# pangenome/impg

Hardware: AMD Instinct MI355X
Metric: projected ranges/sec, 1M-PAF 100k-BED -x depth 3; CPU coitrees baseline (higher is better)
Workload: dtype int32

## Files before the change

impg_amd/csrc/kernels.hip:

```cpp
#include <hip/hip_runtime.h>

#include <cstring>

#include "device_prims.hpp"
#include "impg_internal.hpp"
#include "kernels.hpp"

namespace impg {

__device__ __forceinline__ unsigned lane_id() { return threadIdx.x & 63u; }
__device__ __forceinline__ unsigned long long lanemask_lt() { return (1ull << lane_id()) - 1ull; }

template <int CTRL, int ROW_MASK>
__device__ __forceinline__ uint32_t dpp_or0(uint32_t x) {
  return (uint32_t)__builtin_amdgcn_update_dpp(0, (int)x, CTRL, ROW_MASK, 0xF, false);
}
__device__ __forceinline__ uint32_t wave_incl_scan(uint32_t x) {
  x += dpp_or0<0x111, 0xF>(x);
  x += dpp_or0<0x112, 0xF>(x);
  x += dpp_or0<0x114, 0xF>(x);
  x += dpp_or0<0x118, 0xF>(x);
  x += dpp_or0<0x142, 0xA>(x);
  x += dpp_or0<0x143, 0xC>(x);
  return x;
// ... 1462 lines not shown
};
constexpr uint32_t PROJ_WL_WORDS = 65u + 3u;
constexpr uint32_t PROJ_RG_WORDS = PROJ_BLOCK + 4u * PROJ_BLOCK + PROJ_WAVES + (4u - PROJ_WAVES % 4u) % 4u;
__device__ __forceinline__ PairIn pair_of_place(uint32_t pp, uint32_t lblock, uint32_t n_pairs, const FrontierRec *__restrict__ fr,
                                                const uint32_t *__restrict__ pair_range, const uint32_t *__restrict__ pair_entry,
                                                const ProjList &pl, const WindowLists &wl, uint32_t *wl_off ) {
  PairIn x;
  x.live = pp < n_pairs;
  x.p = pp; x.eidx = 0xFFFFFFFFu; x.f_start = 0; x.f_end = 0;
  uint32_t r = 0;
  if (wl.tile_first && lblock * PROJ_BLOCK >= n_pairs) {
  } else if (wl.tile_first) {
    const uint32_t pp_last = min(lblock * PROJ_BLOCK + PROJ_BLOCK, n_pairs) - 1u;
    uint32_t base_i = wl.tile_first[lblock], ri = 0, k = 0;
    bool found = !x.live;
    for (;;) {
      if (threadIdx.x < 65u) wl_off[threadIdx.x] = base_i + threadIdx.x < wl.n_fr ? wl.pair_off[base_i + threadIdx.x] : 0xFFFFFFFFu;
      __syncthreads();
      const uint32_t lim = wl_off[64];
      if (!found && pp < lim) {
        uint32_t j = 0;
#pragma unroll
        for (uint32_t st = 32u; st > 0u; st >>= 1) j += wl_off[j + st] <= pp ? st : 0u;
        ri = base_i + j;
        k = pp - wl_off[j];
        found = true;
      }
      __syncthreads();
      if (lim > pp_last) break;
      base_i += 64u;
    }
    if (x.live) {
      const uint4 w = wl.win[ri];
      const FrontierRec sf = wl.se[ri];
      const int2 se = make_int2(sf.start, sf.end);
      x.f_start = se.x; x.f_end = se.y;
      if (w.y - (w.x & ~3u) > 64u) x.eidx = pair_entry[pp];
      else x.eidx = w.x + select_bit64(w.z, w.w, k);
      if (wl.range_out) wl.range_out[pp] = wl.range_places ? ri : wl.perm[ri];
    }
  } else if (x.live) {
    if (pl.slot) { x.p = pl.slot[pp]; r = pl.range[pp]; x.eidx = pl.entry[pp]; }
    else { r = pair_range[pp]; x.eidx = pair_entry[pp]; }
    asm volatile("" : "+v"(r), "+v"(x.eidx));
    const FrontierRec f = fr[r];
    x.f_start = f.start; x.f_end = f.end;
  }
  return x;
}
template <uint32_t NB>
__device__ __forceinline__ void regroup_by_entry(PairIn &x, uint32_t *scratch ) {
  uint4 *rg_pay = reinterpret_cast<uint4 *>(scratch);
  uint32_t *rg_hist = scratch + 4u * NB, *rg_ws = rg_hist + NB;
  rg_hist[threadIdx.x] = 0u;
  __syncthreads();
  const uint32_t bin = x.eidx & (NB - 1u);
  const uint32_t pos = atomicAdd(&rg_hist[bin], 1u);
  __syncthreads();
  {
    const uint32_t cnt = rg_hist[threadIdx.x], inc = wave_incl_scan(cnt);
    if (lane_id() == 63u) rg_ws[threadIdx.x >> 6] = inc;
    __syncthreads();
    uint32_t base = 0;
#pragma unroll
    for (uint32_t k = 0; k + 1u < NB / 64u; k++) base += k < (threadIdx.x >> 6) ? rg_ws[k] : 0u;
    rg_hist[threadIdx.x] = base + inc - cnt;
  }
  __syncthreads();
  rg_pay[rg_hist[bin] + pos] = make_uint4(x.eidx, x.p, (uint32_t)x.f_start, (uint32_t)x.f_end);
  __syncthreads();
  const uint4 mine = rg_pay[threadIdx.x];
  x.eidx = mine.x; x.p = mine.y; x.f_start = (int32_t)mine.z; x.f_end = (int32_t)mine.w;
  x.live = x.eidx != 0xFFFFFFFFu;
}
template <uint32_t NW>
__device__ __forceinline__ void count_accepted(uint32_t mine, unsigned long long *__restrict__ accepted, uint32_t *wcnt ) {
  uint32_t w = mine;
#pragma unroll
  for (int o = 32; o > 0; o >>= 1) w += __shfl_xor(w, o);
  if (lane_id() == 0) wcnt[threadIdx.x >> 6] = w;
  __syncthreads();
  if (threadIdx.x == 0) {
    uint32_t tot = 0;
#pragma unroll
    for (uint32_t k = 0; k < NW; k++) tot += wcnt[k];
    if (tot) atomicAdd(&accepted[(blockIdx.x % COUNT_SLOTS) * COUNT_STRIDE], (unsigned long long)tot);
  }
}
template <bool TRANSITIVE, int MODE>
__global__ __launch_bounds__(PROJ_BLOCK) void project_kernel(DeviceIndexView v, const FrontierRec *__restrict__ fr,
                                                      const uint32_t *__restrict__ pair_range,
                                                      const uint32_t *__restrict__ pair_entry, uint32_t n_pairs,
                                                      HitArrays h, unsigned long long *__restrict__ accepted,
                                                      uint32_t *__restrict__ err_flag, double min_identity,
                                                      SliceArrays sl, ProjList pl, int xcd_map,
                                                      const uint32_t *__restrict__ n_pairs_dev, int regroup, WindowLists wl) {
  if (n_pairs_dev) n_pairs = *n_pairs_dev;
  const uint32_t per_xcd = gridDim.x >> 3;
  const uint32_t lblock = xcd_map ? (blockIdx.x & 7u) * per_xcd + (blockIdx.x >> 3) : blockIdx.x;
  const uint32_t pp = lblock * PROJ_BLOCK + threadIdx.x;
#ifdef IMPG_PHASE_CLOCKS
  unsigned long long phase_t[10];
  for (int i = 0; i < 10; i++) phase_t[i] = 0;
  PHASE_MARK(0);
#endif
  bool ok = false;
  TileScan res;
  res.found = res.any = false;
  res.pqs = res.pts = res.pqe = res.pte = -1;
  uint32_t qid = HIT_NONE;
  __shared__ uint32_t wl_off[PROJ_WL_WORDS];
  __shared__ uint4 rg_scratch[PROJ_RG_WORDS / 4u];
  __shared__ uint32_t wcnt[PROJ_WAVES];
  PairIn x = pair_of_place(pp, lblock, n_pairs, fr, pair_range, pair_entry, pl, wl, wl_off);
  PHASE_MARK(1);
  if (regroup) regroup_by_entry<PROJ_BLOCK>(x, reinterpret_cast<uint32_t *>(rg_scratch));
  PHASE_MARK(2);
  if (x.live) {
    project_pair<TRANSITIVE, MODE>(v, x.eidx, x.f_start, x.f_end, x.p, min_identity, err_flag, sl, accepted, ok, qid, res PHASE_PASS);
    h.qid[x.p] = qid;
    if (ok) {
      h.c[x.p] = make_int4(res.pqs, res.pqe, res.pts, res.pte);
    }
  }
  PHASE_MARK(7);
  count_accepted<PROJ_WAVES>(ok ? 1u : 0u, accepted, wcnt);
#ifdef IMPG_PHASE_CLOCKS
  PHASE_MARK(8);
  if ((blockIdx.x & 63u) == 0u && lane_id() == 0u && phase_t[3] && phase_t[4] && phase_t[5] && phase_t[6]) {
    for (int i = 0; i < 8; i++) atomicAdd(&g_phase_clk[i], phase_t[i + 1] - phase_t[i]);
    atomicAdd(&g_phase_clk[15], 1ull);
  }
#endif
}

#ifndef IMPG_STG_THREADS
#define IMPG_STG_THREADS 512
#endif
#ifndef IMPG_STG_RANGES
#define IMPG_STG_RANGES 256
#endif
#ifndef IMPG_STG_ECAP
#define IMPG_STG_ECAP 56
#endif
constexpr uint32_t STG_THREADS = IMPG_STG_THREADS, STG_WAVES = STG_THREADS / 64u;
constexpr uint32_t STG_RANGES = IMPG_STG_RANGES;
constexpr uint32_t STG_ECAP = IMPG_STG_ECAP;
constexpr uint32_t STG_ENT_V4 = STG_ECAP * STG_ENT_STRIDE / 4u;
constexpr uint32_t STG_LINE_V4 = STG_ECAP * STG_REC_STRIDE / 4u;
static_assert((STG_RANGES & (STG_RANGES - 1u)) == 0u && STG_RANGES < STG_THREADS && STG_THREADS % 64u == 0, "a thread per range, whole waves");
static_assert(STG_LINE_V4 * 4u >= 5u * STG_THREADS + STG_WAVES, "the unstaged path's scratch overlays the line buffer");
static_assert(STG_ECAP * 4u <= STG_THREADS, "one pass copies the entries");
constexpr int OUT_SLOTS = 0, OUT_QS = 1, OUT_ROWS = 2;
template <bool TRANSITIVE, bool MASKS, bool CAN_STAGE = true, uint32_t NR = STG_RANGES, uint32_t NT = STG_THREADS, int MODE = 0, int OUT = OUT_SLOTS>
__device__ __forceinline__ uint32_t project_places(const DeviceIndexView &v, const uint32_t *__restrict__ pair_entry, const HitArrays &h,
                                                   unsigned long long *__restrict__ accepted, uint32_t *__restrict__ err_flag,
                                                   const WindowLists &wl, uint32_t r0, uint32_t P0, uint32_t P1, uint32_t emin, uint32_t n_e,
                                                   bool regroup_all, const uint32_t *st_off, const uint4 *st_win, const int2 *st_se,
                                                   const uint4 *st_ent, uint4 *st_line PHASE_ARG, double min_identity = 0.0,
                                                   const uint32_t *st_dest = nullptr, const uint32_t *st_tid = nullptr) {
  const SliceArrays no_sl{nullptr, nullptr, nullptr, nullptr};
  uint32_t n_ok = 0;
  constexpr bool ordered = OUT == OUT_ROWS;
  constexpr bool qs = OUT == OUT_QS;
  if (ordered || qs) regroup_all = false;
  uint32_t e_next = 0xFFFFFFFFu;
  if (!MASKS && (unsigned long long)P0 + threadIdx.x < P1) e_next = pair_entry[P0 + threadIdx.x];
  const bool by_visit = ordered && MASKS && wl.ord.by_visit != 0u;
  uint32_t v_next = 0u;
  if (by_visit && (unsigned long long)P0 + threadIdx.x < P1) v_next = wl.ord.vpos[P0 + threadIdx.x];
#pragma unroll 1
  for (uint32_t base = P0; base < P1; base += NT) {
    if (base + NT < base) break;
    const uint32_t pp = base + threadIdx.x;
    PairIn y;
    y.live = pp < P1 ? 1u : 0u;
    y.p = pp; y.eidx = 0xFFFFFFFFu; y.f_start = 0; y.f_end = 0;
    uint32_t j = 0;
#pragma unroll
    for (uint32_t st = NR / 2u; st > 0u; st >>= 1) j += st_off[j + st] <= pp ? st : 0u;
    uint32_t o_dest = 0, o_tid = 0;
    if (y.live) {
      const int2 se = st_se[j];
      y.f_start = se.x; y.f_end = se.y;
      if (MASKS) {
        const uint4 w = st_win[j];
        const bool listed = w.y - (w.x & ~3u) > 64u;
        if (listed) y.eidx = pair_entry[pp];
        else if (by_visit) y.eidx = w.x + v_next;
        else y.eidx = w.x + select_bit64(w.z, w.w, pp - st_off[j]);
        if (ordered) {
          o_dest = st_dest[j] + (listed || by_visit ? pp - st_off[j] : (uint32_t)wl.ord.vpos[pp]);
          o_tid = st_tid ? st_tid[j] : wl.se[r0 + j].target_id;
        } else if (qs) o_tid = r0 + j;
        else if (wl.range_out) wl.range_out[pp] = wl.range_places ? r0 + j : wl.perm[r0 + j];
      } else {
        y.eidx = e_next;
      }
    }
    if (!MASKS) {
      e_next = 0xFFFFFFFFu;
      if ((unsigned long long)pp + NT < P1) e_next = pair_entry[pp + NT];
    }
    if (by_visit) {
      v_next = 0u;
      if ((unsigned long long)pp + NT < P1) v_next = wl.ord.vpos[pp + NT];
    }
    if (regroup_all) regroup_by_entry<NT>(y, reinterpret_cast<uint32_t *>(st_line));
    if (y.live) {
      bool ok = false;
      TileScan res;
      res.found = res.any = false;
      res.pqs = res.pts = res.pqe = res.pte = -1;
      uint32_t qid = HIT_NONE;
      const uint32_t slot = y.eidx - emin;
      const uint4 *se = st_ent + min(slot, STG_ECAP - 1u) * (STG_ENT_STRIDE / 4u);
      if (CAN_STAGE && slot < n_e && (se[1].z & OP_LEN_MASK) <= INLINE_TILES * TILE_OPS)
        project_pair<TRANSITIVE, MODE, true>(v, y.eidx, y.f_start, y.f_end, y.p, min_identity, err_flag, no_sl, accepted, ok, qid, res PHASE_PASS, se,
                                             reinterpret_cast<const uint32_t *>(st_line + slot * (STG_REC_STRIDE / 4u)));
      else
        project_pair<TRANSITIVE, MODE>(v, y.eidx, y.f_start, y.f_end, y.p, min_identity, err_flag, no_sl, accepted, ok, qid, res PHASE_PASS);
      if (ordered) put_ordered_row(wl.ord, o_dest, qid, o_tid, ok, res.pqs, res.pqe, res.pts, res.pte);
      else {
        if (qs) reinterpret_cast<uint2 *>(h.qid)[y.p] = make_uint2(qid, o_tid);
        else h.qid[y.p] = qid;
        if (ok) h.c[y.p] = make_int4(res.pqs, res.pqe, res.pts, res.pte);
      }
      n_ok += ok ? 1u : 0u;
    }
    if (regroup_all) __syncthreads();
  }
  return n_ok;
}
template <bool TRANSITIVE, bool MASKS, int OUT = OUT_SLOTS>
__global__ __launch_bounds__(STG_THREADS) void project_staged_kernel(DeviceIndexView v, const uint32_t *__restrict__ pair_entry,
                                                      uint32_t n_pairs, HitArrays h, unsigned long long *__restrict__ accepted,
                                                      uint32_t *__restrict__ err_flag, int regroup, WindowLists wl) {
  const uint32_t per_xcd = gridDim.x >> 3;
  const uint32_t sblock = (blockIdx.x & 7u) * per_xcd + (blockIdx.x >> 3);
  __shared__ uint4 st_ent[STG_ENT_V4];
  __shared__ uint4 st_line[STG_LINE_V4];
  __shared__ uint4 st_win[STG_RANGES];
  __shared__ int2 st_se[STG_RANGES];
  __shared__ uint32_t st_off[STG_RANGES + 4u];
  __shared__ uint32_t st_dest[OUT == OUT_ROWS ? STG_RANGES : 1u], st_tid[OUT == OUT_ROWS ? STG_RANGES : 1u];
  __shared__ uint32_t wred[2u * STG_WAVES];
  __shared__ uint32_t wcnt[STG_WAVES];
  const uint32_t r0 = sblock * STG_RANGES;
  if (r0 >= wl.n_fr) return;
  const uint32_t nr = min(STG_RANGES, wl.n_fr - r0);
  if (OUT == OUT_ROWS && threadIdx.x < nr) st_dest[threadIdx.x] = wl.ord.dest[r0 + threadIdx.x];
#ifdef IMPG_PHASE_CLOCKS
  unsigned long long stg_t[8], phase_t[10];
#define STG_MARK(i) do { asm volatile("s_waitcnt vmcnt(0) lgkmcnt(0)" ::: "memory"); stg_t[i] = __builtin_readcyclecounter(); } while (0)
#else
#define STG_MARK(i) do { } while (0)
#endif
  STG_MARK(0);
  uint32_t emin = 0xFFFFFFFFu, emax = 0u;
  if (threadIdx.x <= STG_RANGES) {
    uint32_t o = 0xFFFFFFFFu;
    if (threadIdx.x < nr) o = wl.pair_off[r0 + threadIdx.x];
    else if (threadIdx.x == nr) o = r0 + nr < wl.n_fr ? wl.pair_off[r0 + nr] : n_pairs;
    st_off[threadIdx.x] = o;
    if (threadIdx.x < nr) {
      const uint4 w = wl.win[r0 + threadIdx.x];
      st_win[threadIdx.x] = w;
      { const FrontierRec sf = wl.se[r0 + threadIdx.x]; st_se[threadIdx.x] = make_int2(sf.start, sf.end); if (OUT == OUT_ROWS) st_tid[threadIdx.x] = sf.target_id; }
      if (w.y - (w.x & ~3u) > 64u) { emin = w.x; emax = w.y - 1u; }
      else if (w.z | w.w) {
        emin = w.x + (w.z ? (uint32_t)__builtin_ctz(w.z) : 32u + (uint32_t)__builtin_ctz(w.w));
        emax = w.x + (w.w ? 63u - (uint32_t)__builtin_clz(w.w) : 31u - (uint32_t)__builtin_clz(w.z));
      }
    }
  }
  {
#pragma unroll
    for (int o = 32; o > 0; o >>= 1) {
      emin = min(emin, (uint32_t)__shfl_xor((int)emin, o));
      emax = max(emax, (uint32_t)__shfl_xor((int)emax, o));
    }
    if (lane_id() == 0) { wred[threadIdx.x >> 6] = emin; wred[STG_WAVES + (threadIdx.x >> 6)] = emax; }
    __syncthreads();
#pragma unroll
    for (uint32_t k = 0; k < STG_WAVES; k++) { emin = min(emin, wred[k]); emax = max(emax, wred[STG_WAVES + k]); }
  }
  const uint32_t P0 = st_off[0], P1 = st_off[nr];
  uint32_t n_ok = 0;
  STG_MARK(1);
  const bool sparse = emin <= emax && emax - emin >= 4u * STG_ECAP;
  uint32_t n_e = 0;
  if (emin <= emax && !sparse) {
    n_e = min(STG_ECAP, emax - emin + 1u);
    if (threadIdx.x < n_e * 4u) st_ent[(threadIdx.x >> 2) * (STG_ENT_STRIDE / 4u) + (threadIdx.x & 3u)] = reinterpret_cast<const uint4 *>(v.entries + emin)[threadIdx.x];
    __syncthreads();
    const uint32_t w = threadIdx.x >> 6, l = lane_id();
    constexpr uint32_t TURNS = (STG_ECAP + STG_WAVES - 1u) / STG_WAVES;
    uint4 buf[TURNS];
#pragma unroll
    for (uint32_t k = 0; k < TURNS; k++) {
      const uint32_t i = w + k * STG_WAVES;
      buf[k] = make_uint4(0u, 0u, 0u, 0u);
      if (i < n_e) {
        const uint4 e1 = st_ent[i * (STG_ENT_STRIDE / 4u) + 1u];
        const uint32_t n = e1.z & OP_LEN_MASK, m = (n + TILE_OPS - 1u) / TILE_OPS;
        if (m <= INLINE_TILES && (l >> 3) < m) buf[k] = reinterpret_cast<const uint4 *>(v.pfx + (size_t)e1.y * TILE_WORDS)[l];
      }
    }
#pragma unroll
    for (uint32_t k = 0; k < TURNS; k++) {
      const uint32_t i = w + k * STG_WAVES;
      if (i < n_e) st_line[i * (STG_REC_STRIDE / 4u) + (l >> 3) * (STG_LINE_STRIDE / 4u) + (l & 7u)] = buf[k];
    }
    __syncthreads();
  }
  STG_MARK(2);
  n_ok = project_places<TRANSITIVE, MASKS, true, STG_RANGES, STG_THREADS, 0, OUT>(v, pair_entry, h, accepted, err_flag, wl, r0, P0, P1, emin, n_e,
                                                                                  sparse && regroup != 0, st_off, st_win, st_se, st_ent, st_line PHASE_PASS,
                                                                                  0.0, st_dest, OUT == OUT_ROWS ? st_tid : nullptr);
#ifdef IMPG_PHASE_CLOCKS
  STG_MARK(3);
  if ((blockIdx.x & 15u) == 0u && threadIdx.x == 0u) {
    if (sparse) {
      atomicAdd(&g_phase_clk[13], stg_t[3] - stg_t[0]);
      atomicAdd(&g_phase_clk[14], 1ull);
      atomicAdd(&g_phase_clk[12], (unsigned long long)(emax - emin));
    } else {
      for (int i = 0; i < 3; i++) atomicAdd(&g_phase_clk[i], stg_t[i + 1] - stg_t[i]);
      atomicAdd(&g_phase_clk[9], (unsigned long long)(P1 - P0));
      atomicAdd(&g_phase_clk[10], emin <= emax && emax - emin >= STG_ECAP ? 1ull : 0ull);
      atomicAdd(&g_phase_clk[15], 1ull);
      atomicAdd(&g_phase_clk[11], emin <= emax ? (unsigned long long)(emax - emin + 1u) : 0ull);
    }
  }
#endif
  count_accepted<STG_WAVES>(n_ok, accepted, wcnt);
}
#undef STG_MARK

#ifndef IMPG_ENT_RANGES
#define IMPG_ENT_RANGES 512
#endif
#ifndef IMPG_ENT_THREADS
#define IMPG_ENT_THREADS 256
#endif
constexpr uint32_t ENT_RANGES = IMPG_ENT_RANGES;
constexpr uint32_t ENT_THREADS = IMPG_ENT_THREADS, ENT_WAVES = ENT_THREADS / 64u;
constexpr uint32_t ENT_REC_STRIDE = ENT_CP_OFF + 16u;
static_assert((ENT_RANGES & (ENT_RANGES - 1u)) == 0u && ENT_RANGES % ENT_THREADS == 0 && ENT_THREADS % 64u == 0, "whole turns of the block over its ranges");
constexpr uint32_t ENT_REC_V4 = ENT_WAVES * ENT_REC_STRIDE / 4u, ENT_LIST_V4 = ENT_WAVES * ENT_RANGES * 2u / 16u;
static_assert((ENT_REC_V4 + ENT_LIST_V4) * 4u >= 5u * ENT_THREADS + ENT_WAVES, "the unstaged path's scratch overlays the waves' records and lists");
#ifndef IMPG_ENT_WAVES
#define IMPG_ENT_WAVES 6
#endif
template <bool TRANSITIVE, int ORIENT, int MODE, int OUT>
__device__ __forceinline__ void project_entry_chunk(const DeviceIndexView &v, uint4 e0, uint4 e1, uint4 e2, uint4 e3, uint32_t eidx, bool live,
                                                    int32_t f_start, int32_t f_end, uint32_t p, const uint32_t *rec, const HitArrays &h,
                                                    unsigned long long *__restrict__ accepted, uint32_t *__restrict__ err_flag,
                                                    uint32_t &n_ok PHASE_ARG, double min_identity, const OrderedOut &ord, uint32_t tid) {
  const SliceArrays no_sl{nullptr, nullptr, nullptr, nullptr};
  if (live) {
    bool ok = false;
    TileScan res;
    res.found = res.any = false;
    res.pqs = res.pts = res.pqe = res.pte = -1;
    uint32_t qid = HIT_NONE;
    if (ORIENT >= 0) {
      e0 = reinterpret_cast<const uint4 *>(__builtin_assume_aligned(rec, 16))[ENT_CP_OFF / 4u + 3u];
      asm volatile("" : "+v"(e0.x), "+v"(e0.y), "+v"(e0.z), "+v"(e0.w));
    }
    if (ORIENT >= 0)
      project_core<TRANSITIVE, MODE, true, ORIENT>(v, e0, e1, e2, e3, f_start, f_end, p, min_identity, err_flag, no_sl, accepted, ok, qid, res PHASE_PASS, rec);
    else
      project_pair<TRANSITIVE, MODE>(v, eidx, f_start, f_end, p, min_identity, err_flag, no_sl, accepted, ok, qid, res PHASE_PASS);
    if (OUT == OUT_ROWS) put_ordered_row(ord, p, qid, tid, ok, res.pqs, res.pqe, res.pts, res.pte);
    else {
      if (OUT == OUT_QS) reinterpret_cast<uint2 *>(h.qid)[p] = make_uint2(qid, tid);
      else h.qid[p] = qid;
      if (ok) h.c[p] = make_int4(res.pqs, res.pqe, res.pts, res.pte);
    }
    n_ok += ok ? 1u : 0u;
  }
}
#ifndef IMPG_ENT_SLICE_PAIRS
#define IMPG_ENT_SLICE_PAIRS 32768
#endif
constexpr uint32_t ENT_SLICE_PAIRS = IMPG_ENT_SLICE_PAIRS, ENT_MAX_SLICES = 64u;
#ifndef IMPG_ENT_SPARSE
#define IMPG_ENT_SPARSE 4
#endif
constexpr uint32_t ENT_SPARSE = IMPG_ENT_SPARSE;
struct EntSlices {
  uint32_t *work;
  uint32_t *alloc;
  uint32_t cap;
  int phase;
};
template <bool TRANSITIVE, int MODE, int OUT>
__global__ __launch_bounds__(ENT_THREADS) __attribute__((amdgpu_waves_per_eu(IMPG_ENT_WAVES, IMPG_ENT_WAVES)))
void project_entries_kernel(DeviceIndexView v, const uint32_t *__restrict__ pair_entry, uint32_t n_pairs,
                                                      HitArrays h, unsigned long long *__restrict__ accepted,
                                                      uint32_t *__restrict__ err_flag, int regroup, WindowLists wl, double min_identity, EntSlices sl) {
  const uint32_t per_xcd = gridDim.x >> 3;
  uint32_t sblock = (blockIdx.x & 7u) * per_xcd + (blockIdx.x >> 3);
  uint32_t slice = 0u, n_slices = 1u;
  if (sl.phase) {
    if (blockIdx.x >= min(sl.work[0], sl.cap)) return;
    const uint32_t item = sl.work[1u + blockIdx.x];
    sblock = item >> 12; slice = (item >> 6) & 63u; n_slices = (item & 63u) + 1u;
  }
  __shared__ uint4 st_work[ENT_REC_V4 + ENT_LIST_V4];
  uint4 (*st_rec)[ENT_REC_STRIDE / 4u] = reinterpret_cast<uint4 (*)[ENT_REC_STRIDE / 4u]>(st_work);
  uint16_t (*st_list)[ENT_RANGES] = reinterpret_cast<uint16_t (*)[ENT_RANGES]>(st_work + ENT_REC_V4);
  __shared__ uint4 st_win[ENT_RANGES];
  __shared__ int2 st_se[ENT_RANGES];
  __shared__ uint32_t st_off[ENT_RANGES + 4u];
  __shared__ uint16_t st_wide[ENT_RANGES];
  __shared__ uint32_t st_dest[OUT == OUT_ROWS ? ENT_RANGES : 1u];
  constexpr bool ordered = OUT == OUT_ROWS;
  constexpr bool qs = OUT == OUT_QS;
  constexpr bool WIDE_LISTED = ordered;
  __shared__ uint32_t st_nwide, st_alloc, st_next;
  __shared__ uint32_t wred[2u * ENT_WAVES];
  __shared__ uint32_t wcnt[ENT_WAVES];
  const uint32_t r0 = sblock * ENT_RANGES;
  if (r0 >= wl.n_fr) return;
  const uint32_t nr = min(ENT_RANGES, wl.n_fr - r0);
  const uint32_t wv = (uint32_t)__builtin_amdgcn_readfirstlane((int)(threadIdx.x >> 6)), l = lane_id();
#ifdef IMPG_PHASE_CLOCKS
  unsigned long long stg_t[8], phase_t[10];
#define STG_MARK(i) do { asm volatile("s_waitcnt vmcnt(0) lgkmcnt(0)" ::: "memory"); stg_t[i] = __builtin_readcyclecounter(); } while (0)
#else
#define STG_MARK(i) do { } while (0)
#endif
  STG_MARK(0);
  if (threadIdx.x == 0) { st_nwide = 0u; st_alloc = 0u; st_next = 0u; }
  __syncthreads();
  uint32_t emin = 0xFFFFFFFFu, emax = 0u;
#pragma unroll
  for (uint32_t t = threadIdx.x; t < ENT_RANGES; t += ENT_THREADS) {
    if (t < nr) st_off[t] = wl.pair_off[r0 + t];
    else st_off[t + 1u] = 0xFFFFFFFFu;
    if (t == 0) st_off[nr] = r0 + nr < wl.n_fr ? wl.pair_off[r0 + nr] : n_pairs;
    uint32_t glo = 0xFFFFFFFFu, ghi = 0u;
    if (t < nr) {
      const uint4 w = wl.win[r0 + t];
      st_win[t] = w;
      { const FrontierRec sf = wl.se[r0 + t]; st_se[t] = make_int2(sf.start, sf.end); }
      if (ordered) st_dest[t] = wl.ord.dest[r0 + t];
      if (w.y - (w.x & ~3u) > 64u) {
        if (WIDE_LISTED) st_wide[atomicAdd(&st_nwide, 1u)] = (uint16_t)t;
        else if (w.x < w.y) { glo = w.x; ghi = w.y - 1u; emin = min(emin, glo); emax = max(emax, ghi); }
      } else if (w.z | w.w) {
        glo = w.x + (w.z ? (uint32_t)__builtin_ctz(w.z) : 32u + (uint32_t)__builtin_ctz(w.w));
        ghi = w.x + (w.w ? 63u - (uint32_t)__builtin_clz(w.w) : 31u - (uint32_t)__builtin_clz(w.z));
        emin = min(emin, glo);
        emax = max(emax, ghi);
      }
    }
  }
  {
#pragma unroll
    for (int o = 32; o > 0; o >>= 1) {
      emin = min(emin, (uint32_t)__shfl_xor((int)emin, o));
      emax = max(emax, (uint32_t)__shfl_xor((int)emax, o));
    }
    if (l == 0) { wred[wv] = emin; wred[ENT_WAVES + wv] = emax; }
    __syncthreads();
#pragma unroll
    for (uint32_t k = 0; k < ENT_WAVES; k++) { emin = min(emin, wred[k]); emax = max(emax, wred[ENT_WAVES + k]); }
    emin = (uint32_t)__builtin_amdgcn_readfirstlane((int)emin);
    emax = (uint32_t)__builtin_amdgcn_readfirstlane((int)emax);
  }
  const uint32_t P0 = st_off[0], P1 = st_off[nr];
  const bool compact = !ordered;
  uint32_t n_ok = 0;
  STG_MARK(1);
  const bool sparse = emin <= emax && (unsigned long long)(P1 - P0) < (unsigned long long)ENT_SPARSE * (emax - emin + 1u);
  if (!sl.phase && sl.work && !sparse && emin <= emax && P1 - P0 > ENT_SLICE_PAIRS && (uint32_t)__builtin_amdgcn_readfirstlane((int)st_nwide) == 0u) {
    n_slices = min(ENT_MAX_SLICES, (P1 - P0 + ENT_SLICE_PAIRS - 1u) / ENT_SLICE_PAIRS);
    if (threadIdx.x == 0) {
      const uint32_t at = atomicAdd(&sl.work[0], n_slices - 1u);
      for (uint32_t k = 1; k < n_slices; k++)
        if (at + k - 1u < sl.cap) sl.work[1u + at + k - 1u] = sblock << 12 | k << 6 | (n_slices - 1u);
    }
  }
  if (sparse) {
    n_ok = project_places<TRANSITIVE, true, false, ENT_RANGES, ENT_THREADS, MODE, OUT>(v, pair_entry, h, accepted, err_flag, wl, r0, P0, P1, emin, 0u, regroup != 0, st_off, st_win,
                                                               st_se, nullptr, st_work PHASE_PASS, min_identity, st_dest);
  } else if (emin <= emax) {
    const uint4 *ents = reinterpret_cast<const uint4 *>(v.entries);
    const uint4 zero4 = make_uint4(0u, 0u, 0u, 0u);
    const uint32_t n_span = emax - emin + 1u;
    auto take = [&]() -> uint32_t {
      uint32_t i = 0;
      if (l == 0) i = atomicAdd(&st_next, 1u);
      i = (uint32_t)__builtin_amdgcn_readfirstlane((int)i);
      return n_slices > 1u ? min(n_span, slice + i * n_slices) : i;
    };
    uint32_t ic = take(), in = take();
    uint4 cq = zero4, nq = zero4, lc = zero4;
    auto fetch_entry = [&](uint32_t i) -> uint4 {
      uint4 q = zero4;
      if (i < n_span && l < 4u) q = ents[(size_t)(emin + i) * 4u + l];
      return q;
    };
#define IMPG_RDL(x, j) (uint32_t)__builtin_amdgcn_readlane((int)(x), j)
    auto fetch_record = [&](const uint4 &q) -> uint4 {
      uint4 r = zero4;
      const uint32_t nz = IMPG_RDL(q.z, 1), ny = IMPG_RDL(q.y, 1);
      const uint32_t m = ((nz & OP_LEN_MASK) + TILE_OPS - 1u) / TILE_OPS;
      if (m <= INLINE_TILES && (l >> 3) < m) r = reinterpret_cast<const uint4 *>(v.pfx + (size_t)ny * TILE_WORDS)[l];
      return r;
    };
    cq = fetch_entry(ic);
    nq = fetch_entry(in);
    if (ic < n_span) lc = fetch_record(cq);
#pragma unroll 1
    while (ic < n_span) {
      const uint32_t eidx = emin + ic;
      __builtin_amdgcn_wave_barrier();
      st_rec[wv][(l >> 3) * (STG_LINE_STRIDE / 4u) + (l & 7u)] = lc;
      if (l < 4u) st_rec[wv][ENT_CP_OFF / 4u + ((l + 3u) & 3u)] = cq;
      uint4 e0, e1, e2, e3;
      e0.x = IMPG_RDL(cq.x, 0); e0.y = IMPG_RDL(cq.y, 0); e0.z = IMPG_RDL(cq.z, 0); e0.w = IMPG_RDL(cq.w, 0);
      e1.x = IMPG_RDL(cq.x, 1); e1.y = IMPG_RDL(cq.y, 1); e1.z = IMPG_RDL(cq.z, 1); e1.w = IMPG_RDL(cq.w, 1);
      e2.x = IMPG_RDL(cq.x, 2); e2.y = IMPG_RDL(cq.y, 2); e2.z = IMPG_RDL(cq.z, 2); e2.w = IMPG_RDL(cq.w, 2);
      e3.x = IMPG_RDL(cq.x, 3); e3.y = IMPG_RDL(cq.y, 3); e3.z = IMPG_RDL(cq.z, 3); e3.w = IMPG_RDL(cq.w, 3);
      ic = in;
      cq = nq;
      lc = zero4;
      if (ic < n_span) {
        lc = fetch_record(cq);
        in = take();
        nq = fetch_entry(in);
      }
      uint32_t cnt = 0;
      const int32_t e_end = TRANSITIVE ? ((int32_t)e0.x < (int32_t)e0.y ? (int32_t)e0.y : (-2147483647 - 1)) : (int32_t)e0.y;
#pragma unroll
      for (uint32_t q = 0; q < ENT_RANGES / 64u; q++) {
        const uint32_t r = q * 64u + l;
        bool hit = false;
        if (r < nr) {
          const uint4 w = st_win[r];
          const uint32_t d = eidx - w.x;
          if (w.y - (w.x & ~3u) <= 64u) hit = d < 64u && (((d < 32u ? w.z >> d : w.w >> (d - 32u)) & 1u) != 0u);
          else if (!WIDE_LISTED) hit = eidx >= w.x && eidx < w.y && window_hit<TRANSITIVE>(e_end, st_se[r].x);
        }
        const unsigned long long b = __ballot(hit);
        if (hit) st_list[wv][cnt + (uint32_t)__popcll(b & lanemask_lt())] = (uint16_t)r;
        cnt += (uint32_t)__popcll(b);
      }
      uint32_t run = 0;
      if (compact) {
        if (l == 0) run = n_slices > 1u ? atomicAdd(&sl.alloc[sblock], cnt) : atomicAdd(&st_alloc, cnt);
        run = P0 + (uint32_t)__builtin_amdgcn_readfirstlane((int)run);
      }
      asm volatile("s_waitcnt lgkmcnt(0)" ::: "memory");
      __builtin_amdgcn_wave_barrier();
      const uint32_t *rec = reinterpret_cast<const uint32_t *>(&st_rec[wv][0]);
      const int orient = (e1.z & OP_LEN_MASK) > INLINE_TILES * TILE_OPS ? -1 : !(e1.z & EF_REVERSED) ? 0 : (e1.z & EF_STRAND) ? 2 : 1;
      uint32_t tid = 0;
      if (ordered && cnt) tid = wl.se[r0 + (uint32_t)__builtin_amdgcn_readfirstlane((int)st_list[wv][0])].target_id;
#pragma unroll 1
      for (uint32_t k0 = 0; k0 < cnt; k0 += 64u) {
        const bool live = k0 + l < cnt;
        const uint32_t r = live ? (uint32_t)st_list[wv][k0 + l] : 0u;
        const int2 se = st_se[r];
        uint32_t p = run + k0 + l;
        if (!compact) {
          const uint4 w = st_win[r];
          const uint32_t d = eidx - w.x;
          const uint32_t below = d < 32u ? (uint32_t)__popc(w.z & ((1u << d) - 1u))
                                         : (uint32_t)__popc(w.z) + (uint32_t)__popc(w.w & ((1u << (d - 32u)) - 1u));
          p = st_off[r] + below;
        }
        if (ordered) {
          if (live) p = st_dest[r] + (uint32_t)wl.ord.vpos[p];
        } else if (qs) tid = r0 + r;
        else if (live && wl.range_out) wl.range_out[p] = wl.range_places ? r0 + r : wl.perm[r0 + r];
        if (orient == 0) project_entry_chunk<TRANSITIVE, 0, MODE, OUT>(v, e0, e1, e2, e3, eidx, live, se.x, se.y, p, rec, h, accepted, err_flag, n_ok PHASE_PASS, min_identity, wl.ord, tid);
        else if (orient == 1) project_entry_chunk<TRANSITIVE, 1, MODE, OUT>(v, e0, e1, e2, e3, eidx, live, se.x, se.y, p, rec, h, accepted, err_flag, n_ok PHASE_PASS, min_identity, wl.ord, tid);
        else if (orient == 2) project_entry_chunk<TRANSITIVE, 2, MODE, OUT>(v, e0, e1, e2, e3, eidx, live, se.x, se.y, p, rec, h, accepted, err_flag, n_ok PHASE_PASS, min_identity, wl.ord, tid);
        else project_entry_chunk<TRANSITIVE, -1, MODE, OUT>(v, e0, e1, e2, e3, eidx, live, se.x, se.y, p, rec, h, accepted, err_flag, n_ok PHASE_PASS, min_identity, wl.ord, tid);
      }
    }
#undef IMPG_RDL
#ifdef IMPG_PHASE_CLOCKS
    STG_MARK(2);
    if ((blockIdx.x & 15u) == 0u && threadIdx.x == 0u) {
      atomicAdd(&g_phase_clk[0], stg_t[1] - stg_t[0]);
      atomicAdd(&g_phase_clk[2], stg_t[2] - stg_t[1]);
      atomicAdd(&g_phase_clk[9], (unsigned long long)(P1 - P0));
      atomicAdd(&g_phase_clk[15], 1ull);
      atomicAdd(&g_phase_clk[11], (unsigned long long)(emax - emin + 1u));
    }
#endif
  }
  if (!sparse) {
    const SliceArrays no_sl{nullptr, nullptr, nullptr, nullptr};
    const uint32_t nw = st_nwide;
#pragma unroll 1
    for (uint32_t k = 0; k < nw; k++) {
      const uint32_t r = st_wide[k];
      const uint32_t a = st_off[r], b = st_off[r + 1u];
      const int2 se = st_se[r];
#pragma unroll 1
      for (uint32_t pp = a + threadIdx.x; pp < b; pp += ENT_THREADS) {
        bool ok = false;
        TileScan res;
        res.found = res.any = false;
        res.pqs = res.pts = res.pqe = res.pte = -1;
        uint32_t qid = HIT_NONE;
        project_pair<TRANSITIVE, MODE>(v, pair_entry[pp], se.x, se.y, pp, min_identity, err_flag, no_sl, accepted, ok, qid, res PHASE_PASS);
        if (ordered)
          put_ordered_row(wl.ord, st_dest[r] + (pp - a), qid, wl.se[r0 + r].target_id, ok, res.pqs, res.pqe, res.pts, res.pte);
        else {
          if (qs) reinterpret_cast<uint2 *>(h.qid)[pp] = make_uint2(qid, r0 + r);
          else h.qid[pp] = qid;
          if (ok) h.c[pp] = make_int4(res.pqs, res.pqe, res.pts, res.pte);
        }
        n_ok += ok ? 1u : 0u;
        if (wl.range_out && !ordered && !qs) wl.range_out[pp] = wl.range_places ? r0 + r : wl.perm[r0 + r];
      }
    }
  }
#ifdef IMPG_PHASE_CLOCKS
  if (sparse && (blockIdx.x & 15u) == 0u && threadIdx.x == 0u) {
    STG_MARK(3);
    atomicAdd(&g_phase_clk[13], stg_t[3] - stg_t[0]);
    atomicAdd(&g_phase_clk[14], 1ull);
    atomicAdd(&g_phase_clk[12], (unsigned long long)(emax - emin));
  }
#endif
  count_accepted<ENT_WAVES>(n_ok, accepted, wcnt);
}
#undef STG_MARK
#ifdef IMPG_PHASE_CLOCKS
extern "C" void impg_gpu_debug_phase_clocks(unsigned long long *out) {
  unsigned long long z[16] = {};
  (void)hipDeviceSynchronize();
  (void)hipMemcpyFromSymbol(out, HIP_SYMBOL(g_phase_clk), sizeof(z));
  (void)hipMemcpyToSymbol(HIP_SYMBOL(g_phase_clk), z, sizeof(z));
}
#endif

__device__ __forceinline__ int32_t tp_refine(int32_t query_pos, int32_t query_delta, int32_t seg_start, int32_t overlap_pos,
                                             int32_t abs_target_delta, bool first, int32_t lo, int32_t hi) {
  int32_t refined;
  if (abs_target_delta == 0) {
    refined = first ? query_pos : query_pos + query_delta;
  } else {
    const double target_fraction = (double)(overlap_pos - seg_start) / (double)abs_target_delta;
    const double indel_ratio = (double)query_delta / (double)abs_target_delta;
    const double query_advance = target_fraction * (double)abs_target_delta * indel_ratio;
    const double r = round(query_advance);
    const int32_t adv = r >= 2147483647.0 ? 2147483647 : r <= -2147483648.0 ? (-2147483647 - 1) : (int32_t)r;
    refined = (int32_t)((uint32_t)query_pos + (uint32_t)adv);
  }
  return min(max(refined, lo), hi);
}
template <bool TRANSITIVE>
__global__ __launch_bounds__(256) void project_tp_kernel(DeviceIndexView v, const FrontierRec *__restrict__ fr,
                                                         const uint32_t *__restrict__ pair_range,
                                                         const uint32_t *__restrict__ pair_entry, uint32_t n_pairs,
                                                         HitArrays h, unsigned long long *__restrict__ accepted,
                                                         uint32_t *__restrict__ err_flag, double min_identity, int use_ident,
                                                         ProjList pl, const uint32_t *__restrict__ n_pairs_dev) {
  if (n_pairs_dev) n_pairs = *n_pairs_dev;
  const uint32_t per_xcd = gridDim.x >> 3;
  const uint32_t lblock = (blockIdx.x & 7u) * per_xcd + (blockIdx.x >> 3);
  const uint32_t pp = lblock * 256u + threadIdx.x;
  bool ok = false;
  if (pp < n_pairs) {
    const uint32_t p = pl.slot ? pl.slot[pp] : pp;
    const uint32_t r = pl.slot ? pl.range[pp] : pair_range[p];
    const FrontierRec f = fr[r];
    const uint4 *ep = reinterpret_cast<const uint4 *>(v.entries + (pl.slot ? pl.entry[pp] : pair_entry[p]));
    const uint4 e0 = ep[0], e1 = ep[1];
    const int32_t m_ts = (int32_t)e0.x, m_te = (int32_t)e0.y, m_qs = (int32_t)e0.z, m_qe = (int32_t)e0.w;
    const uint32_t n = e1.z & OP_LEN_MASK;
    const bool is_reverse = (e1.z & EF_STRAND) != 0, reversed_entry = (e1.z & EF_REVERSED) != 0;
    int32_t rs = f.start, re = f.end;
    if (TRANSITIVE) { rs = max(rs, m_ts); re = min(re, m_te); }
    uint32_t qid = HIT_NONE;
    int4 out = make_int4(0, 0, 0, 0);
    if (!(m_ts >= re || m_te <= rs) && n) {
      const uint4 *B = reinterpret_cast<const uint4 *>(v.ops) + e1.y;
      const int sdir = reversed_entry ? 1 : (is_reverse ? -1 : 1);
      const int pdir = reversed_entry ? (is_reverse ? -1 : 1) : 1;
      const int32_t s0 = reversed_entry ? m_ts : (is_reverse ? m_te : m_ts);
      const int32_t p0 = reversed_entry ? (is_reverse ? m_qe : m_qs) : m_qs;
      const int64_t x_lo = sdir > 0 ? (int64_t)rs - s0 : (int64_t)s0 - re, x_hi = sdir > 0 ? (int64_t)re - s0 : (int64_t)s0 - rs;
      auto S = [&](uint32_t k) -> int64_t { const uint4 b = B[k]; return (int64_t)(reversed_entry ? b.y : b.x); };
      uint32_t lo = 1, hi = n + 1;
      while (lo < hi) { const uint32_t mid = (lo + hi) >> 1; if (S(mid) <= x_lo) lo = mid + 1; else hi = mid; }
      const uint32_t first = lo - 1;
      lo = 0; hi = n;
      while (lo < hi) { const uint32_t mid = (lo + hi) >> 1; if (S(mid) < x_hi) lo = mid + 1; else hi = mid; }
      if (first < n && lo > 0 && first <= lo - 1) {
        const uint32_t last = lo - 1;
        const uint4 bf0 = B[first], bf1 = B[first + 1], bl0 = B[last], bl1 = B[last + 1];
        auto seg = [&](const uint4 &a, const uint4 &b, int32_t &ppos, int32_t &pdelta, int32_t &sstart, int32_t &send, int32_t &asd) {
          const int32_t sa = (int32_t)(reversed_entry ? a.y : a.x), sb = (int32_t)(reversed_entry ? b.y : b.x);
          const int32_t ja = (int32_t)(reversed_entry ? a.x : a.y), jb = (int32_t)(reversed_entry ? b.x : b.y);
          const int32_t pa = s0 + sdir * sa, pb = s0 + sdir * sb;
          sstart = min(pa, pb); send = max(pa, pb); asd = sb - sa;
          ppos = p0 + pdir * ja; pdelta = pdir * (jb - ja);
        };
        const int32_t qlo = min(m_qs, m_qe), qhi = max(m_qs, m_qe);
        int32_t ppos, pdelta, sstart, send, asd;
        seg(bf0, bf1, ppos, pdelta, sstart, send, asd);
        const int32_t refined_first = tp_refine(ppos, pdelta, sstart, max(sstart, rs), asd, true, qlo, qhi);
        seg(bl0, bl1, ppos, pdelta, sstart, send, asd);
        const int32_t refined_last = tp_refine(ppos, pdelta, sstart, min(send, re), asd, false, qlo, qhi);
        bool keep = true;
        if (use_ident) {
          const int64_t mm = (int64_t)bl1.z - bf0.z, xx = (int64_t)bl1.w - bf0.w;
          const int64_t total = mm + xx;
          const double ident = total == 0 ? 0.0 : (double)mm / (double)total;
          keep = !(ident < min_identity);
        }
        if (keep) {
          if (refined_first < 0 || refined_last < 0) atomicOr(err_flag, 2u);
          const bool swap_q = is_reverse && !reversed_entry;
          out = make_int4(swap_q ? refined_last : refined_first, swap_q ? refined_first : refined_last, rs, re);
          qid = e1.x;
          ok = true;
        }
      }
    }
    h.qid[p] = qid;
    if (ok) h.c[p] = out;
  }
  __shared__ uint32_t wcnt[4];
  unsigned long long m = __ballot(ok);
  if (lane_id() == 0) wcnt[threadIdx.x >> 6] = __popcll(m);
  __syncthreads();
  if (threadIdx.x == 0) {
    uint32_t tot = wcnt[0] + wcnt[1] + wcnt[2] + wcnt[3];
    if (tot) atomicAdd(&accepted[(blockIdx.x % COUNT_SLOTS) * COUNT_STRIDE], (unsigned long long)tot);
  }
}

__global__ __launch_bounds__(256) void slice_counts_kernel(HitArrays h, SliceArrays sl, uint32_t n_pairs,
                                                           uint32_t *__restrict__ cnt) {
  const uint32_t p = blockIdx.x * 256u + threadIdx.x;
  if (p >= n_pairs) return;
  cnt[p] = h.qid[p] == HIT_NONE ? 0u : sl.n[p];
}
__global__ __launch_bounds__(64) void slice_write_kernel(DeviceIndexView v, const uint32_t *__restrict__ pair_entry,
                                                         HitArrays h, SliceArrays sl, uint32_t n_pairs,
// ... 2756 lines not shown
```

Baseline: 68.93 billion.

## Shrink entry kernel LDS footprint to fit six waves per SIMD

Replaces the per-range 16-byte window record in shared memory with a 4-byte low index, an 8-byte mask and a one-bit wide flag. For the unordered forms, the place offsets now overlay the wave scratch buffer and are loaded only when the sparse path needs them. Slice size is tied to range count, and static asserts check that blocks fit a CU's LDS at the requested waves per EU. The ordered-rows form falls back to fewer waves if its LDS does not fit. The intent is higher occupancy, at the cost of extra bit-tests and a ballot per range.

```diff
diff --git a/impg_amd/csrc/kernels.hip b/impg_amd/csrc/kernels.hip
--- a/impg_amd/csrc/kernels.hip
+++ b/impg_amd/csrc/kernels.hip
@@ -1638,13 +1638,14 @@
 static_assert(STG_LINE_V4 * 4u >= 5u * STG_THREADS + STG_WAVES, "the unstaged path's scratch overlays the line buffer");
 static_assert(STG_ECAP * 4u <= STG_THREADS, "one pass copies the entries");
 constexpr int OUT_SLOTS = 0, OUT_QS = 1, OUT_ROWS = 2;
-template <bool TRANSITIVE, bool MASKS, bool CAN_STAGE = true, uint32_t NR = STG_RANGES, uint32_t NT = STG_THREADS, int MODE = 0, int OUT = OUT_SLOTS>
+template <bool TRANSITIVE, bool MASKS, bool CAN_STAGE = true, uint32_t NR = STG_RANGES, uint32_t NT = STG_THREADS, int MODE = 0, int OUT = OUT_SLOTS, bool WIN3 = false>
 __device__ __forceinline__ uint32_t project_places(const DeviceIndexView &v, const uint32_t *__restrict__ pair_entry, const HitArrays &h,
                                                    unsigned long long *__restrict__ accepted, uint32_t *__restrict__ err_flag,
                                                    const WindowLists &wl, uint32_t r0, uint32_t P0, uint32_t P1, uint32_t emin, uint32_t n_e,
                                                    bool regroup_all, const uint32_t *st_off, const uint4 *st_win, const int2 *st_se,
                                                    const uint4 *st_ent, uint4 *st_line PHASE_ARG, double min_identity = 0.0,
-                                                   const uint32_t *st_dest = nullptr, const uint32_t *st_tid = nullptr) {
+                                                   const uint32_t *st_dest = nullptr, const uint32_t *st_tid = nullptr,
+                                                   const uint32_t *st_lo = nullptr, const uint2 *st_mask = nullptr, const uint32_t *st_wbits = nullptr) {
   const SliceArrays no_sl{nullptr, nullptr, nullptr, nullptr};
   uint32_t n_ok = 0;
   constexpr bool ordered = OUT == OUT_ROWS;
@@ -1670,11 +1671,20 @@
       const int2 se = st_se[j];
       y.f_start = se.x; y.f_end = se.y;
       if (MASKS) {
-        const uint4 w = st_win[j];
-        const bool listed = w.y - (w.x & ~3u) > 64u;
+        uint32_t w_lo, m_lo, m_hi;
+        bool listed;
+        if (WIN3) {
+          const uint2 m = st_mask[j];
+          w_lo = st_lo[j]; m_lo = m.x; m_hi = m.y;
+          listed = ((st_wbits[j >> 5] >> (j & 31u)) & 1u) != 0u;
+        } else {
+          const uint4 w = st_win[j];
+          w_lo = w.x; m_lo = w.z; m_hi = w.w;
+          listed = w.y - (w.x & ~3u) > 64u;
+        }
         if (listed) y.eidx = pair_entry[pp];
-        else if (by_visit) y.eidx = w.x + v_next;
-        else y.eidx = w.x + select_bit64(w.z, w.w, pp - st_off[j]);
+        else if (by_visit) y.eidx = w_lo + v_next;
+        else y.eidx = w_lo + select_bit64(m_lo, m_hi, pp - st_off[j]);
         if (ordered) {
           o_dest = st_dest[j] + (listed || by_visit ? pp - st_off[j] : (uint32_t)wl.ord.vpos[pp]);
           o_tid = st_tid ? st_tid[j] : wl.se[r0 + j].target_id;
@@ -1835,7 +1845,19 @@
 constexpr uint32_t ENT_REC_STRIDE = ENT_CP_OFF + 16u;
 static_assert((ENT_RANGES & (ENT_RANGES - 1u)) == 0u && ENT_RANGES % ENT_THREADS == 0 && ENT_THREADS % 64u == 0, "whole turns of the block over its ranges");
 constexpr uint32_t ENT_REC_V4 = ENT_WAVES * ENT_REC_STRIDE / 4u, ENT_LIST_V4 = ENT_WAVES * ENT_RANGES * 2u / 16u;
-static_assert((ENT_REC_V4 + ENT_LIST_V4) * 4u >= 5u * ENT_THREADS + ENT_WAVES, "the unstaged path's scratch overlays the waves' records and lists");
+constexpr uint32_t ENT_OFF_AT = (5u * ENT_THREADS + ENT_WAVES + 3u) & ~3u;
+static_assert((ENT_REC_V4 + ENT_LIST_V4) * 4u >= ENT_OFF_AT + ENT_RANGES + 4u, "the unstaged path's scratch and place offsets overlay the waves' records and lists");
+static_assert(ENT_RANGES <= 65536u, "st_list / st_wide name a range of the block in 16 bits");
+constexpr uint32_t ent_lds_bytes(bool ordered) {
+  return (ENT_REC_V4 + ENT_LIST_V4) * 16u + ENT_RANGES * (4u + 8u + 8u) + ENT_RANGES / 8u + 3u * 4u + 4u * ENT_WAVES * 4u +
+         (ordered ? (ENT_RANGES + 4u) * 4u + ENT_RANGES * 4u + ENT_RANGES * 2u : 4u + 4u + 2u);
+}
+constexpr uint32_t ENT_CU_LDS = 160u * 1024u, ENT_LDS_MARGIN = 2048u;
+constexpr uint32_t ENT_CU_BLOCKS = 6u * 4u / ENT_WAVES;
+constexpr int ENT_ROWS_WAVES = ent_lds_bytes(true) <= ENT_CU_LDS / ENT_CU_BLOCKS ? 6 : 4;
+static_assert(24u % ENT_WAVES == 0u, "whole blocks in a CU's 24 waves");
+static_assert(ent_lds_bytes(false) + ENT_LDS_MARGIN <= ENT_CU_LDS / ENT_CU_BLOCKS, "the timed forms' blocks fill a CU to 6 waves a SIMD");
+static_assert(ent_lds_bytes(true) + ENT_LDS_MARGIN <= ENT_CU_LDS / ((uint32_t)ENT_ROWS_WAVES * 4u / ENT_WAVES), "the ordered-rows form's blocks fill a CU to its waves a SIMD");
 #ifndef IMPG_ENT_WAVES
 #define IMPG_ENT_WAVES 6
 #endif
@@ -1869,7 +1891,7 @@
   }
 }
 #ifndef IMPG_ENT_SLICE_PAIRS
-#define IMPG_ENT_SLICE_PAIRS 32768
+#define IMPG_ENT_SLICE_PAIRS (64 * IMPG_ENT_RANGES)
 #endif
 constexpr uint32_t ENT_SLICE_PAIRS = IMPG_ENT_SLICE_PAIRS, ENT_MAX_SLICES = 64u;
 #ifndef IMPG_ENT_SPARSE
@@ -1883,7 +1905,7 @@
   int phase;
 };
 template <bool TRANSITIVE, int MODE, int OUT>
-__global__ __launch_bounds__(ENT_THREADS) __attribute__((amdgpu_waves_per_eu(IMPG_ENT_WAVES, IMPG_ENT_WAVES)))
+__global__ __launch_bounds__(ENT_THREADS) __attribute__((amdgpu_waves_per_eu(OUT == OUT_ROWS ? ENT_ROWS_WAVES : IMPG_ENT_WAVES, OUT == OUT_ROWS ? ENT_ROWS_WAVES : IMPG_ENT_WAVES)))
 void project_entries_kernel(DeviceIndexView v, const uint32_t *__restrict__ pair_entry, uint32_t n_pairs,
                                                       HitArrays h, unsigned long long *__restrict__ accepted,
                                                       uint32_t *__restrict__ err_flag, int regroup, WindowLists wl, double min_identity, EntSlices sl) {
@@ -1898,16 +1920,19 @@
   __shared__ uint4 st_work[ENT_REC_V4 + ENT_LIST_V4];
   uint4 (*st_rec)[ENT_REC_STRIDE / 4u] = reinterpret_cast<uint4 (*)[ENT_REC_STRIDE / 4u]>(st_work);
   uint16_t (*st_list)[ENT_RANGES] = reinterpret_cast<uint16_t (*)[ENT_RANGES]>(st_work + ENT_REC_V4);
-  __shared__ uint4 st_win[ENT_RANGES];
+  constexpr bool ordered = OUT == OUT_ROWS;
+  __shared__ uint32_t st_lo[ENT_RANGES];
+  __shared__ uint2 st_mask[ENT_RANGES];
+  __shared__ uint32_t st_wbits[ENT_RANGES / 32u];
   __shared__ int2 st_se[ENT_RANGES];
-  __shared__ uint32_t st_off[ENT_RANGES + 4u];
-  __shared__ uint16_t st_wide[ENT_RANGES];
-  __shared__ uint32_t st_dest[OUT == OUT_ROWS ? ENT_RANGES : 1u];
-  constexpr bool ordered = OUT == OUT_ROWS;
+  __shared__ uint32_t st_off_rows[ordered ? ENT_RANGES + 4u : 1u];
+  uint32_t *st_off = ordered ? st_off_rows : reinterpret_cast<uint32_t *>(st_work) + ENT_OFF_AT;
+  __shared__ uint16_t st_wide[ordered ? ENT_RANGES : 1u];
+  __shared__ uint32_t st_dest[ordered ? ENT_RANGES : 1u];
   constexpr bool qs = OUT == OUT_QS;
   constexpr bool WIDE_LISTED = ordered;
   __shared__ uint32_t st_nwide, st_alloc, st_next;
-  __shared__ uint32_t wred[2u * ENT_WAVES];
+  __shared__ uint32_t wred[3u * ENT_WAVES];
   __shared__ uint32_t wcnt[ENT_WAVES];
   const uint32_t r0 = sblock * ENT_RANGES;
   if (r0 >= wl.n_fr) return;
@@ -1922,19 +1947,29 @@
   STG_MARK(0);
   if (threadIdx.x == 0) { st_nwide = 0u; st_alloc = 0u; st_next = 0u; }
   __syncthreads();
-  uint32_t emin = 0xFFFFFFFFu, emax = 0u;
+  uint32_t emin = 0xFFFFFFFFu, emax = 0u, any_wide = 0u;
+  const uint32_t P_end = r0 + nr < wl.n_fr ? wl.pair_off[r0 + nr] : n_pairs;
+  auto load_offsets = [&]() {
+#pragma unroll
+    for (uint32_t t = threadIdx.x; t < ENT_RANGES; t += ENT_THREADS) {
+      if (t < nr) st_off[t] = wl.pair_off[r0 + t];
+      else st_off[t + 1u] = 0xFFFFFFFFu;
+      if (t == 0) st_off[nr] = P_end;
+    }
+  };
+  if (ordered) load_offsets();
 #pragma unroll
   for (uint32_t t = threadIdx.x; t < ENT_RANGES; t += ENT_THREADS) {
-    if (t < nr) st_off[t] = wl.pair_off[r0 + t];
-    else st_off[t + 1u] = 0xFFFFFFFFu;
-    if (t == 0) st_off[nr] = r0 + nr < wl.n_fr ? wl.pair_off[r0 + nr] : n_pairs;
     uint32_t glo = 0xFFFFFFFFu, ghi = 0u;
+    bool wide = false;
     if (t < nr) {
       const uint4 w = wl.win[r0 + t];
-      st_win[t] = w;
+      wide = w.y - (w.x & ~3u) > 64u;
+      st_lo[t] = w.x;
+      st_mask[t] = wide ? make_uint2(w.y, 0u) : make_uint2(w.z, w.w);
       { const FrontierRec sf = wl.se[r0 + t]; st_se[t] = make_int2(sf.start, sf.end); }
       if (ordered) st_dest[t] = wl.ord.dest[r0 + t];
-      if (w.y - (w.x & ~3u) > 64u) {
+      if (wide) {
         if (WIDE_LISTED) st_wide[atomicAdd(&st_nwide, 1u)] = (uint16_t)t;
         else if (w.x < w.y) { glo = w.x; ghi = w.y - 1u; emin = min(emin, glo); emax = max(emax, ghi); }
       } else if (w.z | w.w) {
@@ -1944,6 +1979,9 @@
         emax = max(emax, ghi);
       }
     }
+    const unsigned long long wb = __ballot(wide);
+    if (l == 0) { st_wbits[t >> 5] = (uint32_t)wb; st_wbits[(t >> 5) + 1u] = (uint32_t)(wb >> 32); }
+    any_wide |= wb != 0ull ? 1u : 0u;
   }
   {
 #pragma unroll
@@ -1951,14 +1989,15 @@
       emin = min(emin, (uint32_t)__shfl_xor((int)emin, o));
       emax = max(emax, (uint32_t)__shfl_xor((int)emax, o));
     }
-    if (l == 0) { wred[wv] = emin; wred[ENT_WAVES + wv] = emax; }
+    if (l == 0) { wred[wv] = emin; wred[ENT_WAVES + wv] = emax; wred[2u * ENT_WAVES + wv] = any_wide; }
     __syncthreads();
 #pragma unroll
-    for (uint32_t k = 0; k < ENT_WAVES; k++) { emin = min(emin, wred[k]); emax = max(emax, wred[ENT_WAVES + k]); }
+    for (uint32_t k = 0; k < ENT_WAVES; k++) { emin = min(emin, wred[k]); emax = max(emax, wred[ENT_WAVES + k]); any_wide |= wred[2u * ENT_WAVES + k]; }
     emin = (uint32_t)__builtin_amdgcn_readfirstlane((int)emin);
     emax = (uint32_t)__builtin_amdgcn_readfirstlane((int)emax);
   }
-  const uint32_t P0 = st_off[0], P1 = st_off[nr];
+  const bool has_wide = (uint32_t)__builtin_amdgcn_readfirstlane((int)any_wide) != 0u;
+  const uint32_t P0 = ordered ? st_off[0] : wl.pair_off[r0], P1 = ordered ? st_off[nr] : P_end;
   const bool compact = !ordered;
   uint32_t n_ok = 0;
   STG_MARK(1);
@@ -1972,8 +2011,12 @@
     }
   }
   if (sparse) {
-    n_ok = project_places<TRANSITIVE, true, false, ENT_RANGES, ENT_THREADS, MODE, OUT>(v, pair_entry, h, accepted, err_flag, wl, r0, P0, P1, emin, 0u, regroup != 0, st_off, st_win,
-                                                               st_se, nullptr, st_work PHASE_PASS, min_identity, st_dest);
+    if (!ordered) {
+      load_offsets();
+      __syncthreads();
+    }
+    n_ok = project_places<TRANSITIVE, true, false, ENT_RANGES, ENT_THREADS, MODE, OUT, true>(v, pair_entry, h, accepted, err_flag, wl, r0, P0, P1, emin, 0u, regroup != 0, st_off, nullptr,
+                                                               st_se, nullptr, st_work PHASE_PASS, min_identity, st_dest, nullptr, st_lo, st_mask, st_wbits);
   } else if (emin <= emax) {
     const uint4 *ents = reinterpret_cast<const uint4 *>(v.entries);
     const uint4 zero4 = make_uint4(0u, 0u, 0u, 0u);
@@ -2028,10 +2071,12 @@
         const uint32_t r = q * 64u + l;
         bool hit = false;
         if (r < nr) {
-          const uint4 w = st_win[r];
-          const uint32_t d = eidx - w.x;
-          if (w.y - (w.x & ~3u) <= 64u) hit = d < 64u && (((d < 32u ? w.z >> d : w.w >> (d - 32u)) & 1u) != 0u);
-          else if (!WIDE_LISTED) hit = eidx >= w.x && eidx < w.y && window_hit<TRANSITIVE>(e_end, st_se[r].x);
+          const uint32_t w_lo = st_lo[r];
+          const uint2 m = st_mask[r];
+          const uint32_t d = eidx - w_lo;
+          hit = d < 64u && (((d < 32u ? m.x >> d : m.y >> (d - 32u)) & 1u) != 0u);
+          if (has_wide && ((st_wbits[q * 2u + (l >> 5)] >> (l & 31u)) & 1u) != 0u)
+            hit = !WIDE_LISTED && eidx >= w_lo && eidx < m.x && window_hit<TRANSITIVE>(e_end, st_se[r].x);
         }
         const unsigned long long b = __ballot(hit);
         if (hit) st_list[wv][cnt + (uint32_t)__popcll(b & lanemask_lt())] = (uint16_t)r;
@@ -2055,10 +2100,10 @@
         const int2 se = st_se[r];
         uint32_t p = run + k0 + l;
         if (!compact) {
-          const uint4 w = st_win[r];
-          const uint32_t d = eidx - w.x;
-          const uint32_t below = d < 32u ? (uint32_t)__popc(w.z & ((1u << d) - 1u))
-                                         : (uint32_t)__popc(w.z) + (uint32_t)__popc(w.w & ((1u << (d - 32u)) - 1u));
+          const uint2 m = st_mask[r];
+          const uint32_t d = eidx - st_lo[r];
+          const uint32_t below = d < 32u ? (uint32_t)__popc(m.x & ((1u << d) - 1u))
+                                         : (uint32_t)__popc(m.x) + (uint32_t)__popc(m.y & ((1u << (d - 32u)) - 1u));
           p = st_off[r] + below;
         }
         if (ordered) {
@@ -2083,7 +2128,7 @@
     }
 #endif
   }
-  if (!sparse) {
+  if (WIDE_LISTED && !sparse) {
     const SliceArrays no_sl{nullptr, nullptr, nullptr, nullptr};
     const uint32_t nw = st_nwide;
 #pragma unroll 1
```

After: 69.34 billion, median of 6. No clear change (+0.6%).
